# ZackAttack614/BlackBird

Hardware: AMD Instinct MI355X
Metric: selfplay_games_per_sec (higher is better)
Workload: dtype f32 (float32 operands split exactly into 3 bf16 values, 6 bf16 MFMA products each, f32 accumulate)

## Files before the change

### blackbird_amd/csrc/engine.hip

```cpp
#include "../../include/blackbird_hip.h"
#include "eval.hip.h"
#include "net.hip.h"
#include "net_x3.hip.h"
#include "gnet.hip.h"
#include "gnet_x3.hip.h"
#include "eval_probe.hip.h"
#include "tree.hip.h"
#include "tree_dc.hip.h"
#include "mega2.hip.h"
#include "mega_dc.hip.h"

#include <cmath>
#include <cstdarg>
#include <cstdio>
#include <cstdlib>
#include <cstring>
#include <string>
#include <type_traits>
#include <vector>

static thread_local std::string g_err;
static int fail(int code, const char *fmt, ...) {
    char buf[512];
    va_list ap;
// ... 154 lines not shown
    bb_game_info info;
    TreeDev dev;
    DCEdges edges;
    int32_t *d_child_action = nullptr;
    NetDev net;
    NetX3 x3 = {nullptr, nullptr, nullptr, nullptr, nullptr};
    size_t x3_bytes = 0;
    bool has_weights = false;
    int net_F = 0, net_C = 0;
    bool general_net = false;
    GNetDev gnet = {};
    GNetX3 gx3 = {nullptr, {nullptr, nullptr}};
    size_t gx3_bytes = 0;
    int gnet_C = 0;
    size_t net_sizes[4] = {0, 0, 0, 0};
    hipStream_t stream = nullptr;
    std::vector<void *> allocs;
    int n_games_target = 0;
    int sims_now = 0;
    size_t node_bytes = 0;
    double *d_u = nullptr;
    int32_t *d_actions = nullptr;
    int n_views = 1;
    TreeDev view[2];
    hipStream_t vstream[2] = {nullptr, nullptr};
    int vround[2] = {0, 0};
    struct {
        int launch_steps = 64, queue_limit_s = 30;
        bool level_budget_set = false;
    } tune;
    size_t eval_cache_bytes = 0;
    int *miss_count = nullptr;
    int *miss_slot = nullptr;
    int miss_next[2] = {0, 0};
    bool mega = false;
    bool async_selfplay = false;
    bool dc_fused = false;
    int round = 0;
    int time_every = 0;
    uint64_t eval_launches = 0;
    std::vector<hipEvent_t> ev_pool;
    size_t ev_used = 0;
};

static hipError_t sync_all(bb_engine *e) {
    if (e->vstream[1]) {
        hipError_t r = hipStreamSynchronize(e->vstream[1]);
        if (r != hipSuccess) return r;
    }
    return hipStreamSynchronize(e->stream);
}

template <class T>
static int dalloc(bb_engine *e, T *&p, size_t count, bool zero = true) {
    void *q = nullptr;
    size_t bytes = count * sizeof(T);
    hipError_t err = hipMalloc(&q, bytes ? bytes : 16);
    if (err != hipSuccess) return fail(BB_ERR_HIP, "hipMalloc(%zu) failed: %s", bytes, hipGetErrorString(err));
    e->allocs.push_back(q);
    if (zero && bytes) {
        err = hipMemsetAsync(q, 0, bytes, e->stream);
        if (err != hipSuccess) return fail(BB_ERR_HIP, "hipMemset failed: %s", hipGetErrorString(err));
    }
    p = (T *)q;
    return 0;
}
// ... 52 lines not shown
template <class G>
static void make_views(bb_engine *e) {
    const TreeDev &d = e->dev;
    int n = d.n_slots;
    for (int v = 0; v < e->n_views; v++) {
        TreeDev w = d;
        int off = v == 0 ? 0 : n / 2;
        int cnt = e->n_views == 1 ? n : (v == 0 ? n / 2 : n - n / 2);
        w.n_slots = cnt;
        w.slot_offset = off;
        w.root += off; w.root_N += off; w.n_nodes += off; w.ply += off; w.sims_left += off; w.pend_leaf += off;
        w.pend_expand += off; w.path_len += off; w.game_lid += off; w.sim_serial += off; w.root_W += off;
        w.root_pp += off; w.path += (size_t)off * G::MAXPATH;
        w.anc += (size_t)off * (d.max_plies + 2); w.anc_len += off; w.top_N += off;
        w.path_N += (size_t)off * G::MAXPATH; w.path_all += (size_t)off * G::MAXPATH; w.path_W += (size_t)off * G::MAXPATH; w.leaf_flags += off;
        w.leaf_state = (char *)d.leaf_state + (size_t)off * sizeof(typename G::State);
        w.leaf_game_id += off; w.leaf_serial += off; w.eval_value += off;
        w.eval_policy += (size_t)off * (G::GID == BB_GAME_DRAGONCHESS ? G::A : G::S);
        w.evals += off; w.ctr += (size_t)off * 8;
        w.nodes = (char *)d.nodes + (size_t)off * d.node_cap * e->node_bytes;
        w.resume_cur += off; w.resume_depth += off; w.post_slot += off; w.post_count += 4 * v;
        e->view[v] = w;
    }
}

static size_t eval_cache_entry_bytes(const bb_config *cfg) { return cfg->game == BB_GAME_DRAGONCHESS ? 128 : 64; }
static int eval_cache_log2_of(const bb_config *cfg) {
    const bool rounds_too = cfg->game == BB_GAME_CONNECT4;
    if ((cfg->game != BB_GAME_CONNECT4 && cfg->game != BB_GAME_DRAGONCHESS) || cfg->mcts_kind != BB_MCTS_DYNAMIC ||
        cfg->evaluator != BB_EVAL_NET || !(cfg->launch == BB_LAUNCH_AUTO || (rounds_too && cfg->launch == BB_LAUNCH_ROUNDS)))
        return 0;
    const char *on = getenv("BB_EVAL_CACHE"), *lg = getenv("BB_EVAL_CACHE_LOG2");
    if (on && atoi(on) == 0) return 0;
    const int k = lg ? atoi(lg) : cfg->game == BB_GAME_DRAGONCHESS ? 24 : 26;
    return k < 10 ? 10 : k > 32 ? 32 : k;
}

static long node_capacity_of(const bb_config *cfg) {
    long cap = cfg->node_capacity > 0 ? cfg->node_capacity : (long)cfg->sims_per_move * cfg->max_plies + 2;
    if (cfg->mcts_kind == BB_MCTS_FIXED && cfg->node_capacity <= 0) cap = cap * cfg->max_depth;
    return cap;
}

template <class G>
static void pool_bytes(const bb_config *cfg, size_t *per_slot, size_t *fixed) {
    constexpr bool DC = G::GID == BB_GAME_DRAGONCHESS;
    constexpr size_t NODE_BYTES = DC ? sizeof(DCNode) : sizeof(DenseNode<typename std::conditional<DC, Connect4, G>::type>);
    const size_t cap = (size_t)node_capacity_of(cfg);
    size_t ps = cap * NODE_BYTES;
    if (DC) ps += cap * 24 * sizeof(DCEdge) + (size_t)G::MAXPATH * 4;
    ps += (size_t)G::MAXPATH * 4 + (DC ? (size_t)G::A : (size_t)G::S) * 4 + (size_t)G::S * 16 + sizeof(typename G::State) + 256;
    bb_game_info gi;
    bb_game_info_get(cfg->game, &gi);
    const size_t ng = (size_t)(cfg->max_games > 0 ? cfg->max_games : cfg->n_slots);
    *per_slot = ps;
    *fixed = ng * ((size_t)(cfg->max_plies + 1) * (size_t)gi.example_bytes + 16) + (64u << 20);
    if (const int k = eval_cache_log2_of(cfg)) *fixed += eval_cache_entry_bytes(cfg) << k;
}

static int check_config(const bb_config *cfg) {
    if (!cfg) return fail(BB_ERR_ARG, "null argument");
    if (cfg->n_slots <= 0) return fail(BB_ERR_ARG, "n_slots must be positive");
    if (cfg->mcts_kind == BB_MCTS_FIXED && cfg->max_depth <= 0)
        return fail(BB_ERR_ARG, "MaxDepth for MCTS must be > 0.");
    if (cfg->sims_per_move < 0 || cfg->max_plies <= 0) return fail(BB_ERR_ARG, "bad sims_per_move/max_plies");
    int ndev = bb_device_count();
    if (ndev <= 0) return fail(BB_ERR_HIP, "no HIP device available (this library has no CPU fallback)");
// ... 71 lines not shown
    d.lid_stride = cfg->n_slots;
    auto env_int = [](const char *name, int dflt) {
        const char *v = getenv(name);
        return v ? atoi(v) : dflt;
    };
    if (int v = env_int("BB_LEVEL_BUDGET", 0); v >= 1) {
        d.level_budget = v;
        e->tune.level_budget_set = true;
    }
    e->tune.launch_steps = env_int("BB_LAUNCH_STEPS", 64);
    e->tune.queue_limit_s = env_int("BB_QUEUE_LIMIT_S", 30);
    if (cfg->launch < 0 || cfg->launch > BB_LAUNCH_ROUNDS || cfg->net_form < 0 || cfg->net_form > BB_NET_FORM_SPLIT) {
        delete e;
        return fail(BB_ERR_ARG, "bad bb_config.launch / net_form");
    }
    e->async_selfplay = cfg->game != BB_GAME_DRAGONCHESS && cfg->mcts_kind == BB_MCTS_DYNAMIC &&
                        cfg->evaluator != BB_EVAL_ROLLOUT && cfg->launch != BB_LAUNCH_LOCKSTEP;
    e->mega = e->async_selfplay && cfg->evaluator == BB_EVAL_NET && cfg->launch == BB_LAUNCH_AUTO;
    e->dc_fused = cfg->game == BB_GAME_DRAGONCHESS && cfg->mcts_kind == BB_MCTS_DYNAMIC && cfg->evaluator == BB_EVAL_NET &&
                  cfg->launch == BB_LAUNCH_AUTO;
    if (int v = env_int("BB_TREE_GPW", 0); v >= 1 && v <= 64 / e->info.S) d.gpw = v;
    d.temp = 1.0;
    GAME_SWITCH(cfg->game, rc = engine_alloc<G>(e); break);
    if (!rc) {
        if (const int k = eval_cache_log2_of(cfg)) {
            uint8_t *tab = nullptr;
            e->eval_cache_bytes = eval_cache_entry_bytes(cfg) << k;
            rc = dalloc(e, tab, e->eval_cache_bytes);
            d.eval_cache = tab;
            d.eval_cache_log2 = k;
        }
    }
    if (!rc) rc = dalloc(e, d.eval_cache_ctr, 2);
    if (!rc && d.eval_cache && e->async_selfplay) rc = dalloc(e, e->miss_count, 8) || dalloc(e, e->miss_slot, (size_t)cfg->n_slots);
    if (rc) {
        bb_destroy(e);
        return rc;
    }
    e->n_views = 1;
    if (e->async_selfplay && !e->mega && cfg->evaluator == BB_EVAL_NET && cfg->n_slots >= 512) e->n_views = 2;
    if (const char *env = getenv("BB_GROUPS")) e->n_views = (atoi(env) == 2 && e->async_selfplay && cfg->n_slots >= 2) ? 2 : 1;
    e->vstream[0] = e->stream;
    if (e->n_views == 2) HIPCHK(hipStreamCreateWithFlags(&e->vstream[1], hipStreamNonBlocking));
    GAME_SWITCH(cfg->game, make_views<G>(e); break);
    *out = e;
    return BB_OK;
}

extern "C" int bb_destroy(bb_engine *e) {
    if (!e) return BB_OK;
    (void)hipSetDevice(e->cfg.device);
    if (e->stream) (void)hipStreamSynchronize(e->stream);
    for (void *p : e->allocs) (void)hipFree(p);
    for (auto ev : e->ev_pool) (void)hipEventDestroy(ev);
    if (e->vstream[1]) {
        (void)hipStreamSynchronize(e->vstream[1]);
        (void)hipStreamDestroy(e->vstream[1]);
    }
    if (e->stream) (void)hipStreamDestroy(e->stream);
    delete e;
    return BB_OK;
}

extern "C" int bb_timing_enable(bb_engine *e, int every_n) {
    if (!e || every_n < 0) return fail(BB_ERR_ARG, "bad arguments");
    HIPCHK(hipSetDevice(e->cfg.device));
    HIPCHK(sync_all(e));
// ... 957 lines not shown
            if (e->x3.w0) {
                if constexpr (G::S <= 8) k_selfplay_queue<G, 8, true, 12><<<nb, 768, 0, e->stream>>>(dm, e->net, e->x3, e->cfg.noise_on, lim, own);
                else k_selfplay_queue<G, 4, true, 8><<<nb, 512, 0, e->stream>>>(dm, e->net, e->x3, e->cfg.noise_on, lim, own);
            } else {
                k_selfplay_queue<G, 8><<<nb, 768, 0, e->stream>>>(dm, e->net, e->x3, e->cfg.noise_on, lim, own);
            }
            HIPCHK(hipGetLastError());
            if (timed) {
                HIPCHK(hipEventRecord(e->ev_pool[e->ev_used + 1], e->stream));
                e->ev_used += 2;
            }
          }
            return BB_OK;
        }
        for (int r = 0; r < rounds; r++) {
            for (int v = 0; v < e->n_views; v++) {
                TreeDev &d = e->view[v];
                hipStream_t st = e->vstream[v];
                int tb = nblk((size_t)((d.n_slots + d.gpw - 1) / d.gpw) * 64);
                int nb = (d.n_slots + 4 * PWMAX - 1) / (4 * PWMAX);
                if (e->n_views == 2) nb = 256 > nb ? 256 : nb;
                int round = e->vround[v]++;
                k_tree_async<G><<<tb, 256, 0, st>>>(d, round);
                HIPCHK(hipGetLastError());
                const typename G::State *ls = (const typename G::State *)d.leaf_state;
                if (d.evaluator == BB_EVAL_NET) {
                    bool timed = v == 0 && e->time_every > 0 && (e->eval_launches++ % (uint64_t)e->time_every) == 0 &&
                                 e->ev_used + 2 <= e->ev_pool.size();
                    if (timed) HIPCHK(hipEventRecord(e->ev_pool[e->ev_used], st));
                    const int *n_ptr = d.post_count + (round & 3), *slot_list = d.post_slot;
                    EvalCache store = {nullptr, 0};
                    if constexpr (G::CACHE_KEY) {
                        if (d.eval_cache && e->miss_count && e->general_net) {
                            store = {(u32x4 *)d.eval_cache, d.eval_cache_log2};
                            int *mc = e->miss_count + 4 * v, *ms = e->miss_slot + d.slot_offset;
                            if (e->miss_next[v] != round)
                                HIPCHK(hipMemsetAsync(mc, 0, 4 * sizeof(int), st));
                            e->miss_next[v] = round + 1;
                            k_eval_cache_probe<G><<<(d.n_slots + 3) / 4, 256, 0, st>>>(e->net, store, n_ptr, slot_list, mc, round, ms, ls,
                                                                                       d.leaf_game_id, d.leaf_serial, e->cfg.noise_on,
                                                                                       d.eval_value, d.eval_policy, G::S, d.evals,
                                                                                       d.eval_cache_ctr);
                            n_ptr = mc + (round & 3);
                            slot_list = ms;
                        }
                    }
                    if (e->general_net) {
                        int rc = launch_gnet<G>(e, d.n_slots, n_ptr, slot_list, ls, nullptr, d.leaf_game_id,
                                                d.leaf_serial, e->cfg.noise_on, d.eval_value, nullptr, d.eval_policy, G::S, st,
                                                d.slot_offset, store);
                        if (rc) return rc;
                    } else if (e->x3.w0) {
                        if constexpr (G::C <= 4)
                            k_net_x3<G><<<(d.n_slots + 3) / 4, 256, 0, st>>>(e->net, e->x3, 0, n_ptr, slot_list, ls,
                                                                              nullptr, d.leaf_game_id, d.leaf_serial, e->cfg.noise_on,
                                                                              d.eval_value, nullptr, d.eval_policy, G::S, store);
                    } else
                    k_net_compact<G, PWMAX><<<nb, 256, 0, st>>>(e->net, n_ptr, slot_list, ls,
                                                                 d.leaf_game_id, d.leaf_serial, e->cfg.noise_on, d.eval_value,
                                                                 d.eval_policy, G::S, store);
                    HIPCHK(hipGetLastError());
                    if (timed) {
                        HIPCHK(hipEventRecord(e->ev_pool[e->ev_used + 1], st));
                        e->ev_used += 2;
                    }
                } else {
                    k_hash_eval<G><<<nblk(d.n_slots), 256, 0, st>>>(d.n_slots, ls, d.leaf_game_id, d.salt, d.salt_per_game,
                                                                    d.first_game_id, d.eval_value, d.eval_policy, G::S);
                    HIPCHK(hipGetLastError());
                }
            }
        }
// ... 260 lines not shown
```

### blackbird_amd/csrc/eval_probe.hip.h

```cpp
#pragma once
#include "net.hip.h"

template <class G>
__global__ void __launch_bounds__(256)
k_eval_cache_probe(NetDev nd, EvalCache cache, const int *n_ptr, const int *slot_list, int *miss_count, int round, int *miss_slot,
                   const typename G::State *states, const uint32_t *game_id, const int32_t *serial, int noise, float *value_out,
                   float *policy_out, int pstride, uint64_t *evals, unsigned long long *ctr) {
    static_assert(G::CACHE_KEY, "a game whose positions have a one-word key (Connect4)");
    __shared__ int s_slot[4], s_probe[4], s_base;
    const int wave = __builtin_amdgcn_readfirstlane(threadIdx.x >> 6), lane = threadIdx.x & 63;
    const int n = *n_ptr, pos = blockIdx.x * 4 + wave;
    const bool live = pos < n;
    const int slot = slot_list[live ? pos : 0];
    const typename G::State st = states[slot];
    const uint64_t key = live ? G::cache_key(st) : 0;
    u32x4 *const entry = eval_cache_entry(cache, key);
    const u32x4 chunk = eval_cache_load(entry, lane);
    if (blockIdx.x == 0 && threadIdx.x == 0) miss_count[(round + 2) & 3] = 0;
    float cv = 0.f, cpr = 0.f;
    const bool hit = eval_cache_hit<G::A>(chunk, key, lane, cv, cpr) && key != 0;
    if (hit) {
        if (lane == 0) {
            value_out[slot] = cv;
            evals[slot] -= 1;
        }
        dense_prior_tail<G>(nd, cpr, slot, true, game_id, serial, noise, policy_out, pstride, lane);
    }
    if (lane == 0) {
        s_slot[wave] = live && !hit ? slot : -1;
        s_probe[wave] = key ? 1 + (int)hit : 0;
    }
    __syncthreads();
    if (threadIdx.x == 0) {
        int n_miss = 0, n_probe = 0, n_hit = 0;
        for (int w = 0; w < 4; w++) {
            n_miss += s_slot[w] >= 0;
            n_probe += s_probe[w] > 0;
            n_hit += s_probe[w] > 1;
        }
        s_base = n_miss ? atomicAdd(&miss_count[round & 3], n_miss) : 0;
        if (n_probe && ctr) {
            if (n_hit) atomicAdd(&ctr[0], (unsigned long long)n_hit);
            atomicAdd(&ctr[1], (unsigned long long)n_probe);
        }
    }
    __syncthreads();
    if (lane == 0 && s_slot[wave] >= 0) {
        int rank = 0;
        for (int w = 0; w < wave; w++) rank += s_slot[w] >= 0;
        miss_slot[s_base + rank] = slot;
    }
}
```

### blackbird_amd/csrc/games.hip.h

```cpp
#pragma once
#include <hip/hip_runtime.h>
#include <stdint.h>

template <class T>
__device__ __forceinline__ T *as_lds(T *p) {
#if __HIP_DEVICE_COMPILE__
    __builtin_assume(__builtin_amdgcn_is_shared((const void *)p));
#endif
    return p;
}
template <class T>
__device__ __forceinline__ T *as_global(T *p) {
#if __HIP_DEVICE_COMPILE__
    __builtin_assume(!__builtin_amdgcn_is_shared((const void *)p) && !__builtin_amdgcn_is_private((const void *)p));
#endif
    return p;
}

struct GridState {
    uint64_t p1, p2;
};
static_assert(sizeof(GridState) == 16, "packed grid state is 16 bytes");

#define BB_HD __host__ __device__ __forceinline__
// ... 115 lines not shown
                for (int r = 0; r < H; r++) col |= 1ull << (r * STR);
                uint64_t cb = (occ >> prev) & col;
                int top = cb ? (63 - bb_clz64(cb)) / STR : 0;
                cell = top * STR + prev;
            } else {
                cell = (prev / W) * STR + (prev % W);
            }
            uint64_t bit = 1ull << cell;
            int p = (b1 & bit) ? 1 : (b2 & bit) ? 2 : 0;
            uint64_t own = p == 1 ? b1 : p == 2 ? b2 : (~occ & board_mask());
            if (win_cells(own) & bit) return p;
        } else {
            uint64_t w1 = win_cells(b1), w2 = win_cells(b2), any = w1 | w2;
            if (any) return (w1 >> bb_ctz64(any)) & 1 ? 1 : 2;
        }
        if (is_over(occ)) return 0;
        return -1;
    }

    BB_HD static void encode_cell(const State &s, int r, int c, int8_t out[3]) {
        int bit = r * STR + c;
        out[0] = (int8_t)((s.p1 >> bit) & 1);
        out[1] = (int8_t)((s.p2 >> bit) & 1);
        out[2] = gs_player(s) == 1 ? 1 : -1;
    }

    static constexpr bool CACHE_KEY = DROP;
    BB_HD static uint64_t cache_key(const State &s) {
        const uint64_t b1 = gs_cells(s.p1), b2 = gs_cells(s.p2), occ = b1 | b2, floor = (1ull << W) - 1;
        const uint64_t above = (occ << STR) | floor;
        if (!DROP || (b1 & b2) || (occ & ~board_mask()) || (occ & ~above)) return 0;
        return b1 | (above & ~occ) | ((uint64_t)(gs_player(s) == 1) << 63);
    }
};

BB_HD uint64_t bb_mix64(uint64_t z) {
    z ^= z >> 33;
    z *= 0xff51afd7ed558ccdull;
    z ^= z >> 33;
    z *= 0xc4ceb9fe1a85ec53ull;
    z ^= z >> 33;
    return z;
}

using Connect4 = GridGame<6, 7, 4, 8, 7, 8, 0>;
using TicTacToe = GridGame<3, 3, 3, 4, 9, 16, 1>;

struct alignas(16) DCState {
    int8_t b[64];
    int8_t player, prev;
    int8_t castle[4];
    int8_t pad[10];
};
static_assert(sizeof(DCState) == 80, "packed DragonChess state is 80 bytes");

struct DCKey {
    uint64_t w[5];
    BB_HD bool none() const { return (w[0] | w[1] | w[2] | w[3] | w[4]) == 0; }
    BB_HD bool operator==(const DCKey &o) const {
        return w[0] == o.w[0] && w[1] == o.w[1] && w[2] == o.w[2] && w[3] == o.w[3] && w[4] == o.w[4];
    }
    BB_HD uint64_t tag() const {
        uint64_t t = bb_mix64(w[0]);
        for (int i = 1; i < 5; i++) t = bb_mix64(t ^ w[i]);
        return t;
    }
};

struct DragonChess {
    static constexpr int H = 8, W = 8, C = 17, A = 4032, S = 144, GID = 2;
    static constexpr int MAXPATH = 128;
    static constexpr bool CELL_BF16 = true;
    static constexpr bool CACHE_KEY = false;
    using State = DCState;

    BB_HD static State initial() {
        State s;
        for (int i = 0; i < 64; i++) s.b[i] = 0;
        const int8_t back[8] = {-5, -3, -4, -6, -1, -4, -3, -5};
// ... 268 lines not shown
```

### blackbird_amd/csrc/net.hip.h

```cpp
#pragma once
#include <type_traits>
#include "games.hip.h"
#include "rng.hip.h"

typedef float f32x4 __attribute__((ext_vector_type(4)));

__device__ __forceinline__ void wave_lds_handover() { __builtin_amdgcn_fence(__ATOMIC_ACQ_REL, "wavefront"); }

struct NetDev {
    int R, D, A;
    const float *w0;
    const f32x4 *wt;
    const float *epi;
    const float *head;
    int head_floats;
    int off_vk, off_v3, off_d1k, off_d1b, off_d2k, off_d2b, off_pk, off_p6, off_pdk, off_pdb;
    uint64_t seed;
    float alpha, eps;
    float inv_alpha, inv_beta;
    int dbg;
};
#ifdef BB_DIAG
#define ND_DBG(bit) (nd.dbg & (bit))
#else
// ... 88 lines not shown
    float sv[NPL];
    float m = -INFINITY;
#pragma unroll
    for (int k0 = 0; k0 < NPL; k0 += UB) {
        float w0[UB], w1[UB], wb[UB];
#pragma unroll
        for (int u = 0; u < UB; u++) {
            const int a = lane + 64 * (k0 + u);
            w0[u] = pdk[a];
            w1[u] = pdk[A + a];
            wb[u] = pdb[a];
        }
#pragma unroll
        for (int u = 0; u < UB; u++) {
            sv[k0 + u] = wide_logit<HW>(h.R0, h.R1, w0[u], w1[u], wb[u]);
            m = fmaxf(m, sv[k0 + u]);
        }
    }
    m = wave_max_f32(m);
    float tot = 0.f;
#pragma unroll
    for (int k = 0; k < NPL; k++) tot += wide_expterm(sv[k], m);
    tot = wave_sum_f32(tot);
    h.m = m;
    h.inv = 1.0f / tot;
}

__device__ __forceinline__ float pooled_sum(float v) { return wave_sum_f32(v); }

typedef unsigned int u32x4 __attribute__((ext_vector_type(4)));
struct EvalCache {
    u32x4 *tab;
    int log2;
};
__device__ __forceinline__ u32x4 *eval_cache_entry(const EvalCache &c, uint64_t key) {
    return c.tab + 4 * (size_t)(bb_mix64(key) >> (64 - c.log2));
}
template <int A>
__device__ __forceinline__ void eval_cache_put(u32x4 *entry, uint64_t key, float value, float pr, int lane) {
    static_assert(A == 7, "an entry holds the value and seven priors");
    const int c = lane < 4 ? lane : 0;
    const float lo = __shfl(pr, c > 0 ? 2 * c - 1 : 0, 64), hi = __shfl(pr, 2 * c, 64);
    if (lane < 4)
        *(__attribute__((address_space(1))) u32x4 *)(void *)(entry + lane) =
            u32x4{(uint32_t)key, (uint32_t)(key >> 32), __float_as_uint(c == 0 ? value : lo), __float_as_uint(hi)};
}
__device__ __forceinline__ u32x4 eval_cache_load(const u32x4 *entry, int lane) {
    u32x4 z = {0u, 0u, 0u, 0u};
    if (lane < 4) z = *(const __attribute__((address_space(1))) u32x4 *)(const void *)(entry + lane);
    return z;
}
template <int A>
__device__ __forceinline__ bool eval_cache_hit(u32x4 ch, uint64_t key, int lane, float &value, float &pr) {
    const bool ok = lane < 4 && ch[0] == (uint32_t)key && ch[1] == (uint32_t)(key >> 32);
    if ((__ballot(ok) & 0xFull) != 0xFull) return false;
    const float f0 = __uint_as_float(ch[2]), f1 = __uint_as_float(ch[3]);
    value = lane_f32(f0, 0);
    const int i = (lane < A ? lane : 0) + 1;
    const float lo = __shfl(f0, i >> 1, 64), hi = __shfl(f1, i >> 1, 64);
    pr = lane < A ? ((i & 1) ? hi : lo) : 0.f;
    return true;
}

__device__ __forceinline__ u32x4 *dc_eval_cache_entry(const EvalCache &c, uint64_t tag) {
    return c.tab + 8 * (size_t)(tag >> (64 - c.log2));
}
__device__ __forceinline__ u32x4 dc_eval_cache_load(const u32x4 *entry, int lane) {
    u32x4 z = {0u, 0u, 0u, 0u};
    if (lane < 8) z = *(const __attribute__((address_space(1))) u32x4 *)(const void *)(entry + lane);
    return z;
}
__device__ __forceinline__ uint64_t dc_key_word(DCKey k, int lane) {
    return lane == 0 ? k.w[0] : lane == 1 ? k.w[1] : lane == 2 ? k.w[2] : lane == 3 ? k.w[3] : k.w[4];
}
__device__ __forceinline__ bool dc_eval_cache_hit(u32x4 ch, DCKey key, uint64_t tag, int lane, WideHead &h) {
    const uint64_t pay = (uint64_t)ch[2] | ((uint64_t)ch[3] << 32);
    const bool ok = lane < 8 && ch[0] == (uint32_t)tag && ch[1] == (uint32_t)(tag >> 32) && (lane >= 5 || pay == dc_key_word(key, lane));
    if ((__ballot(ok) & 0xFFull) != 0xFFull) return false;
    const float f0 = __uint_as_float(ch[2]), f1 = __uint_as_float(ch[3]);
    h.value = lane_f32(f0, 5);
    h.R0 = lane_f32(f1, 5);
    h.R1 = lane_f32(f0, 6);
    h.m = lane_f32(f1, 6);
    h.inv = lane_f32(f0, 7);
    return true;
}
__device__ __forceinline__ void dc_eval_cache_put(u32x4 *entry, DCKey key, uint64_t tag, WideHead h, int lane) {
    const uint64_t kw = dc_key_word(key, lane);
    const uint32_t lo = lane < 5 ? (uint32_t)kw : __float_as_uint(lane == 5 ? h.value : lane == 6 ? h.R1 : h.inv);
    const uint32_t hi = lane < 5 ? (uint32_t)(kw >> 32) : lane == 5 ? __float_as_uint(h.R0) : lane == 6 ? __float_as_uint(h.m) : 0u;
    if (lane < 8)
        *(__attribute__((address_space(1))) u32x4 *)(void *)(entry + lane) = u32x4{(uint32_t)tag, (uint32_t)(tag >> 32), lo, hi};
// ... 92 lines not shown
                    if (lane + 64 * k < A) {
                        sv[k] = (1.0f - nd.eps) * (sv[k] * inv) + nd.eps * bb_beta_noise(nd.seed, gid, ser, (uint32_t)(lane + 64 * k), nd.alpha);
                        t2 += sv[k];
                    }
                t2 = wave_sum_f32(t2);
                inv = 1.0f / t2;
            }
#pragma unroll
            for (int k = 0; k < NPL; k++)
                if (lane + 64 * k < A) outp[lane + 64 * k] = sv[k] * inv;
        }
    } else {
        static_assert(A > 64 || 2 * A <= 64, "the prior-noise draws use two lanes per action");
        const bool act = lane < A;
        const float l = act ? wide_logit<HW>(R0, R1, pdk[act ? lane : 0], pdk[A + (act ? lane : 0)], pdb[act ? lane : 0]) : -INFINITY;
        constexpr bool ROW0 = A <= 16;
        const float m = ROW0 ? row0_max_f32(l) : wave_max_f32(l);
        float pr = act ? wide_expterm(l, m) : 0.f;
        const float tot = ROW0 ? row0_sum_f32(pr) : wave_sum_f32(pr);
        pr = pr * __builtin_amdgcn_rcpf(tot);
        if constexpr (A == 7)
            if (cache_entry) eval_cache_put<A>(cache_entry, cache_key, value, pr, lane);
        if (live && act && logits_out) logits_out[(size_t)pos * A + lane] = l;
        dense_prior_tail<G>(nd, pr, pos, live, game_id, serial, noise, policy_out, pstride, lane);
    }
}

template <class G>
__device__ __forceinline__ u32x4 *eval_cache_store_entry(const EvalCache &store, const typename G::State *states, int pos, bool live,
                                                         uint64_t &key) {
    key = 0;
    if constexpr (G::CACHE_KEY) {
        if (store.tab && states && live) key = G::cache_key(states[pos]);
        if (key) return eval_cache_entry(store, key);
    }
    return nullptr;
}

template <class G, int PW>
__device__ __forceinline__ void net_head_tail(const NetDev &nd, int n, int pos0, const int *slot_list, const float *rv,
                                              const float *rp, const uint32_t *game_id, const int32_t *serial, int noise,
                                              float *value_out, float *logits_out, float *policy_out, int pstride,
                                              WideHead *compact = nullptr, EvalCache store = {nullptr, 0},
                                              const typename G::State *states = nullptr) {
    constexpr int HW = G::H * G::W;
    static_assert(HW <= 64, "one lane per pixel of a position");
    const int lane = threadIdx.x & 63;
    for (int pp = 0; pp < PW; pp++) {
        const bool live = pos0 + pp < n;
        if (!live && !compact) break;
        const int pos = live ? (slot_list ? slot_list[pos0 + pp] : pos0 + pp) : 0;
        const float x = lane < HW ? rv[pp * HW + lane] : 0.f;
        const float x0 = lane < HW ? rp[2 * (pp * HW + lane)] : 0.f, x1 = lane < HW ? rp[2 * (pp * HW + lane) + 1] : 0.f;
        uint64_t ckey;
        u32x4 *centry = eval_cache_store_entry<G>(store, states, pos, live, ckey);
        head_one<G>(nd, pooled_sum(x), pooled_sum(x0), pooled_sum(x1), pos, live, game_id, serial, noise, value_out, logits_out,
                    policy_out, pstride, compact ? compact + pp : nullptr, centry, ckey);
    }
}

template <class G, int PW, int WMODE = 0>
__device__ __forceinline__ void net_body(const NetDev &nd, int n, int pos0, const int *slot_list, float *wlds,
                                         const typename G::State *states, const int8_t *planes,
                                         const uint32_t *game_id, const int32_t *serial, int noise, float *value_out,
                                         float *logits_out, float *policy_out, int pstride, bool zero_lds = true,
                                         WideHead *compact = nullptr, EvalCache store = {nullptr, 0}) {
    using NG = NetGeom<G, PW>;
// ... 356 lines not shown
```

### blackbird_amd/csrc/net_x3.hip.h

```cpp
#pragma once
#include "net.hip.h"

typedef __bf16 bf16x8 __attribute__((ext_vector_type(8)));
typedef short s16x4 __attribute__((ext_vector_type(4)));
typedef unsigned int u32x2 __attribute__((ext_vector_type(2)));
typedef unsigned int u32x4 __attribute__((ext_vector_type(4)));

template <class G>
struct X3Geom {
    static constexpr int H = G::H, W = G::W, CIN = G::C, A = G::A, HW = H * W;
    static_assert(CIN <= 32, "the first conv packs at most 32 input planes per tap");
    static_assert(HW <= 64, "one lane per pixel in the heads");
    static constexpr bool WIDE_IN = CIN > 4;
    static constexpr int RS = W + 1;
    static constexpr int S0 = RS + 1;
    static constexpr bool CONTIG = (16 % RS) == 0;
    static_assert(CONTIG || (W == 8 && H % 2 == 0), "tile shapes exist for 4-, 8- and 9-slot rows");
    static constexpr int NT = CONTIG ? (H * RS + 15) / 16 : H / 2;
    static constexpr bool SWZ = RS == 8;
    static constexpr int SLOT_B = 96;
    static constexpr int SLOTS_BOARD = (H + 2) * RS + 2;
    static constexpr int SLOTS_TILES = CONTIG ? S0 + 16 * NT + RS + 2 : 0;
    static constexpr int SLOTS = SLOTS_BOARD > SLOTS_TILES ? SLOTS_BOARD : SLOTS_TILES;
    static constexpr int X_B = SLOTS * SLOT_B;
// ... 79 lines not shown
__device__ __forceinline__ void net_body_x3(const NetDev &nd, const NetX3 &x3, int n, int pos0, const int *slot_list,
                                            unsigned char *wl, const typename G::State *states, const int8_t *planes,
                                            const uint32_t *game_id, const int32_t *serial, int noise, float *value_out,
                                            float *logits_out, float *policy_out, int pstride, bool zero_lds,
                                            WideHead *compact = nullptr, EvalCache cache = {nullptr, 0}, int *probe_out = nullptr) {
    using XG = X3Geom<G>;
    constexpr int W = XG::W, CIN = XG::CIN, HW = XG::HW, NT = XG::NT, SB = XG::SLOT_B, RS = XG::RS;
    constexpr bool WIDE_IN = XG::WIDE_IN;
    int lane_ = threadIdx.x & 63;
    asm volatile("" : "+v"(lane_));
    const int lane = lane_;
    const int g = lane >> 4, nn = lane & 15, gh = g >> 1, gl = g & 1;
    static_assert(!PP || !WLDS, "the two-buffer form keeps its weights in registers, a layer ahead");
    unsigned char *X = wl;
    unsigned char *X2 = wl + XG::X_B;
    typename G::State *sst = (typename G::State *)(wl + (PP ? 2 : 1) * XG::X_B);
    auto OI = [&](int pos) { return slot_list ? slot_list[pos] : pos; };
    const bool live = pos0 < n;
#ifdef BB_STAMPS_NET
    long long _ns = clock64();
#endif

    const typename G::State *sst_in = sst;
    typename G::State my_state;
    if constexpr (PP) sst_in = as_lds(&states[OI(live ? pos0 : 0)]);
    else my_state = planes ? G::initial() : states[OI(live ? pos0 : 0)];
    static_assert(!CACHE || (G::CACHE_KEY && !PP), "the evaluation cache: Connect4, value and priors formed here");
    uint64_t ckey = 0;
    u32x4 *centry = nullptr;
    u32x4 cchunk = {0u, 0u, 0u, 0u};
    if constexpr (CACHE) {
        if (cache.tab && live && !planes) ckey = G::cache_key(my_state);
        if (ckey) {
            centry = eval_cache_entry(cache, ckey);
            cchunk = eval_cache_load(centry, lane);
        }
        if (probe_out) *probe_out = ckey ? 0 : -1;
    }
    const unsigned char *w0p = x3.w0;
    bf16x8 w0a[WIDE_IN ? 27 : 3];
    bf16x8 w0b;
    if constexpr (WIDE_IN) {
#pragma unroll
        for (int i = 0; i < 27; i++) w0a[i] = WLDS ? *(const bf16x8 *)(w0p + (i * 64 + lane) * 16) : x3_ldg(w0p + (i * 64 + lane) * 16);
    } else {
#pragma unroll
        for (int q = 0; q < 3; q++) w0a[q] = *(const bf16x8 *)(w0p + (q * 64 + lane) * 16);
        w0b = *(const bf16x8 *)(w0p + (3 * 64 + lane) * 16);
    }
    const float *epi = PP ? as_lds(nd.epi) : nd.epi;
    const f32x4 bias0 = *(const f32x4 *)(epi + 4 * g), scale0 = *(const f32x4 *)(epi + 16 + 4 * g),
                shift0 = *(const f32x4 *)(epi + 32 + 4 * g);
    NSUB(5);
    if (zero_lds) {
        u32x4 z = {0u, 0u, 0u, 0u};
        if constexpr (PP) {
            constexpr int NHALO = RS + XG::H + (XG::SLOTS - (XG::H + 1) * RS), CH = SB / 16;
            constexpr int NCH = 2 * NHALO * CH;
#pragma unroll
            for (int k = 0; k < (NCH + 63) / 64; k++) {
                const int i = lane + 64 * k;
                const int buf = i >= NHALO * CH, j = i - buf * NHALO * CH, hs = j / CH, c = j - hs * CH;
                const int slot = hs < RS ? hs : hs < RS + XG::H ? (hs - RS + 1) * RS : (XG::H + 1) * RS + (hs - RS - XG::H);
                if (64 * k + 63 < NCH || i < NCH) *(u32x4 *)(wl + buf * XG::X_B + slot * SB + c * 16) = z;
            }
        } else {
            for (int i = lane; i < XG::WAVE_BYTES / 16; i += 64) ((u32x4 *)wl)[i] = z;
// ... 28 lines not shown
                unsigned b[32];
#pragma unroll
                for (int c = 0; c < 32; c++) b[c] = c < CIN ? __float_as_uint((float)v[c]) >> 16 : 0u;
#pragma unroll
                for (int k = 0; k < 16; k++) pk[k] = b[2 * k] | (b[2 * k + 1] << 16);
            }
            unsigned char *dst = X + ((y + 1) * RS + (x + 1)) * SB;
#pragma unroll
            for (int k = 0; k < 4; k++) *(u32x4 *)(dst + 16 * k) = u32x4{pk[4 * k], pk[4 * k + 1], pk[4 * k + 2], pk[4 * k + 3]};
        }
    } else
    if (lane < HW && live) {
        const int y = lane / W, x = lane % W;
        int8_t v[4] = {0, 0, 0, 0};
        if (planes) {
            const int8_t *src = planes + ((size_t)pos0 * HW + lane) * CIN;
#pragma unroll
            for (int c = 0; c < CIN; c++) v[c] = src[c];
        } else {
            int8_t e[CIN];
            if constexpr (PP) G::encode_cell(*sst_in, y, x, e);
            else G::encode_cell(my_state, y, x, e);
#pragma unroll
            for (int c = 0; c < CIN; c++) v[c] = e[c];
        }
        unsigned b[4];
#pragma unroll
        for (int c = 0; c < 4; c++) b[c] = __float_as_uint((float)v[c]) >> 16;
        *(u32x2 *)(X + ((y + 1) * RS + (x + 1)) * SB) = u32x2{b[0] | (b[1] << 16), b[2] | (b[3] << 16)};
    }
    NSUB(7);
    if constexpr (CACHE) {
        float cv, cpr;
        if (centry && eval_cache_hit<G::A>(cchunk, ckey, lane, cv, cpr)) {
            if (probe_out) *probe_out = 1;
            if (lane == 0 && value_out) value_out[OI(pos0)] = cv;
            dense_prior_tail<G>(nd, cpr, OI(pos0), true, game_id, serial, noise, policy_out, pstride, lane);
            return;
        }
    }
    constexpr int TS = (XG::CONTIG ? 16 : 2 * RS) * SB;
    static_assert(XG::tile_slot(NT - 1, 5) * SB == XG::tile_slot(0, 5) * SB + (NT - 1) * TS && (!XG::SWZ || XG::swz(XG::tile_slot(1, 9)) == XG::swz(XG::tile_slot(0, 9))), "tile stride");
    auto tapoff = [](int tap) { return (tap / 3) * RS + (tap % 3); };
    const int t0off = tapoff(2 * g) * SB, t1off = tapoff(2 * g + 1) * SB;
    const int s0 = XG::tile_slot(0, nn);
    const int aA0 = (s0 - RS - 1 + gh) * SB + ((gl ^ XG::swz(s0 - 1 + gh)) << 4);
    const int aB0 = (s0 + (gh - 1) * RS + 1) * SB + ((gl ^ XG::swz(s0 + 1)) << 4);
    const int aC0 = (s0 + RS + 1) * SB + ((gl ^ XG::swz(s0 + 1)) << 4);
    const int aC1 = aC0 + gh * 32, aC3 = aC0 + (1 - gh) * 64;
    const int aO0 = s0 * SB + ((g ^ (XG::swz(s0) << 1)) << 3);
    const int aH0 = s0 * SB + ((gl ^ XG::swz(s0)) << 4);
    const int aH1 = aH0 + gh * 32, aH3 = aH0 + (1 - gh) * 64;
    const int iA0 = (s0 - RS - 1) * SB;
    bool wv[NT];
#pragma unroll
    for (int t = 0; t < NT; t++) wv[t] = XG::tile_valid(t, nn);
#define aA(t) (aA0 + (t) * TS)
#define aB(t) (aB0 + (t) * TS)
#define aC1(t) (aC1 + (t) * TS)
#define aC3(t) (aC3 + (t) * TS)
#define aO(t) (aO0 + (t) * TS)
#define aH1(t) (aH1 + (t) * TS)
#define aH3(t) (aH3 + (t) * TS)
#define iA(t) (iA0 + (t) * TS)
    wave_lds_handover();
    NSTAMP(0);
    f32x4 acc[NT], sk[NT];
    {
#pragma unroll
        for (int t = 0; t < NT; t++) acc[t] = bias0;
        if constexpr (WIDE_IN) {
#pragma unroll
// ... 324 lines not shown
        const unsigned char *whp = x3.wh;
        const bf16x8 h1 = PP ? x3_ldg(whp + (0 * 64 + lane) * 16) : *(const bf16x8 *)(whp + (0 * 64 + lane) * 16),
                     h2 = PP ? x3_ldg(whp + (1 * 64 + lane) * 16) : *(const bf16x8 *)(whp + (1 * 64 + lane) * 16),
                     h3 = PP ? x3_ldg(whp + (2 * 64 + lane) * 16) : *(const bf16x8 *)(whp + (2 * 64 + lane) * 16);
        const f32x4 hb = {hbias, 0.f, 0.f, 0.f};
        bf16x8 y1[NT], y3[NT];
#pragma unroll
        for (int t = 0; t < NT; t++) {
            y1[t] = *(const bf16x8 *)(X + aH1(t));
            y3[t] = *(const bf16x8 *)(X + aH3(t));
        }
        float xs = 0.f;
#pragma unroll
        for (int t = 0; t < NT; t++) {
            f32x4 a = hb;
            a = __builtin_amdgcn_mfma_f32_16x16x32_bf16(h3, y3[t], a, 0, 0, 0);
            a = __builtin_amdgcn_mfma_f32_16x16x32_bf16(h2, y1[t], a, 0, 0, 0);
            a = __builtin_amdgcn_mfma_f32_16x16x32_bf16(h1, y1[t], a, 0, 0, 0);
            const float v = fmaxf(__builtin_fmaf(a[0], hscale, hshift), 0.f);
            xs += (g < 3 && wv[t]) ? v : 0.f;
        }
        xs += dpp_f32(xs, 0);
        xs += dpp_f32(xs, 1);
        xs += dpp_f32(xs, 2);
        xs += dpp_f32(xs, 3);
        R = lane_f32(xs, 0);
        R0 = lane_f32(xs, 16);
        R1 = lane_f32(xs, 32);
    }
    NSTAMP(3);
    if constexpr (CACHE) {
        if (centry) {
            ckey = G::cache_key(states[OI(pos0)]);
            centry = eval_cache_entry(cache, ckey);
        }
    } else if constexpr (!PP) {
        centry = eval_cache_store_entry<G>(cache, planes ? nullptr : states, live ? OI(pos0) : 0, live, ckey);
    }
    head_one<G>(nd, R, R0, R1, live ? OI(pos0) : 0, live, game_id, serial, noise, value_out,
                logits_out, policy_out, pstride, compact, centry, ckey);
    NSTAMP(4);
}

#undef aA
#undef aB
#undef aC1
#undef aC3
#undef aO
#undef aH1
#undef aH3
#undef iA
template <class G>
__global__ void __launch_bounds__(256) k_net_x3(NetDev nd, NetX3 x3, int n, const int *n_ptr, const int *slot_list, const typename G::State *states,
                                                const int8_t *planes, const uint32_t *game_id, const int32_t *serial, int noise,
                                                float *value_out, float *logits_out, float *policy_out, int pstride, EvalCache store) {
    using XG = X3Geom<G>;
    __shared__ __attribute__((aligned(16))) unsigned char lds[4 * XG::WAVE_BYTES];
    const int wave = threadIdx.x >> 6;
    const int pos0 = blockIdx.x * 4 + wave;
    if (n_ptr) n = *n_ptr;
    if (pos0 >= n) return;
    net_body_x3<G, false>(nd, x3, n, pos0, slot_list, lds + wave * XG::WAVE_BYTES, states, planes, game_id, serial, noise, value_out,
                          logits_out, policy_out, pstride, true, nullptr, store);
}
```

Measured before the change: 9139.

## Make eval cache two-way set associative with stone-count replacement and double its size

Turns the direct-mapped Connect4 evaluation cache into two-way buckets. Probes load both ways (8 lanes), and on a miss a victim way is chosen, preferring an empty way and otherwise the entry with more stones. The chosen way is carried to the store path through a per-slot byte array or LDS, and the default table size doubles. The aim is a higher hit rate so fewer positions need full network evaluations, at the cost of more probe bandwidth, extra ballots and more memory.

```diff
diff --git a/blackbird_amd/csrc/engine.hip b/blackbird_amd/csrc/engine.hip
--- a/blackbird_amd/csrc/engine.hip
+++ b/blackbird_amd/csrc/engine.hip
@@ -210,6 +210,7 @@
     size_t eval_cache_bytes = 0;
     int *miss_count = nullptr;
     int *miss_slot = nullptr;
+    unsigned char *miss_way = nullptr;
     int miss_next[2] = {0, 0};
     bool mega = false;
     bool async_selfplay = false;
@@ -328,7 +329,7 @@
         return 0;
     const char *on = getenv("BB_EVAL_CACHE"), *lg = getenv("BB_EVAL_CACHE_LOG2");
     if (on && atoi(on) == 0) return 0;
-    const int k = lg ? atoi(lg) : cfg->game == BB_GAME_DRAGONCHESS ? 24 : 26;
+    const int k = lg ? atoi(lg) : cfg->game == BB_GAME_DRAGONCHESS ? 24 : 27;
     return k < 10 ? 10 : k > 32 ? 32 : k;
 }
 
@@ -466,7 +467,8 @@
         }
     }
     if (!rc) rc = dalloc(e, d.eval_cache_ctr, 2);
-    if (!rc && d.eval_cache && e->async_selfplay) rc = dalloc(e, e->miss_count, 8) || dalloc(e, e->miss_slot, (size_t)cfg->n_slots);
+    if (!rc && d.eval_cache && e->async_selfplay)
+        rc = dalloc(e, e->miss_count, 8) || dalloc(e, e->miss_slot, (size_t)cfg->n_slots) || dalloc(e, e->miss_way, (size_t)cfg->n_slots);
     if (rc) {
         bb_destroy(e);
         return rc;
@@ -1490,12 +1492,13 @@
                     EvalCache store = {nullptr, 0};
                     if constexpr (G::CACHE_KEY) {
                         if (d.eval_cache && e->miss_count && e->general_net) {
-                            store = {(u32x4 *)d.eval_cache, d.eval_cache_log2};
+                            store = {(u32x4 *)d.eval_cache, d.eval_cache_log2, e->miss_way + d.slot_offset};
                             int *mc = e->miss_count + 4 * v, *ms = e->miss_slot + d.slot_offset;
                             if (e->miss_next[v] != round)
                                 HIPCHK(hipMemsetAsync(mc, 0, 4 * sizeof(int), st));
                             e->miss_next[v] = round + 1;
-                            k_eval_cache_probe<G><<<(d.n_slots + 3) / 4, 256, 0, st>>>(e->net, store, n_ptr, slot_list, mc, round, ms, ls,
+                            k_eval_cache_probe<G><<<(d.n_slots + 3) / 4, 256, 0, st>>>(e->net, store, n_ptr, slot_list, mc, round, ms,
+                                                                                       e->miss_way + d.slot_offset, ls,
                                                                                        d.leaf_game_id, d.leaf_serial, e->cfg.noise_on,
                                                                                        d.eval_value, d.eval_policy, G::S, d.evals,
                                                                                        d.eval_cache_ctr);
diff --git a/blackbird_amd/csrc/eval_probe.hip.h b/blackbird_amd/csrc/eval_probe.hip.h
--- a/blackbird_amd/csrc/eval_probe.hip.h
+++ b/blackbird_amd/csrc/eval_probe.hip.h
@@ -4,6 +4,7 @@
 template <class G>
 __global__ void __launch_bounds__(256)
 k_eval_cache_probe(NetDev nd, EvalCache cache, const int *n_ptr, const int *slot_list, int *miss_count, int round, int *miss_slot,
+                   unsigned char *miss_way,
                    const typename G::State *states, const uint32_t *game_id, const int32_t *serial, int noise, float *value_out,
                    float *policy_out, int pstride, uint64_t *evals, unsigned long long *ctr) {
     static_assert(G::CACHE_KEY, "a game whose positions have a one-word key (Connect4)");
@@ -14,11 +15,12 @@
     const int slot = slot_list[live ? pos : 0];
     const typename G::State st = states[slot];
     const uint64_t key = live ? G::cache_key(st) : 0;
-    u32x4 *const entry = eval_cache_entry(cache, key);
-    const u32x4 chunk = eval_cache_load(entry, lane);
+    u32x4 *const bucket = eval_cache_bucket(cache, key);
+    const u32x4 chunk = eval_cache_load(bucket, lane);
     if (blockIdx.x == 0 && threadIdx.x == 0) miss_count[(round + 2) & 3] = 0;
     float cv = 0.f, cpr = 0.f;
-    const bool hit = eval_cache_hit<G::A>(chunk, key, lane, cv, cpr) && key != 0;
+    int way = 0;
+    const bool hit = eval_cache_hit<G>(chunk, key, lane, cv, cpr, way) && key != 0;
     if (hit) {
         if (lane == 0) {
             value_out[slot] = cv;
@@ -28,6 +30,7 @@
     }
     if (lane == 0) {
         s_slot[wave] = live && !hit ? slot : -1;
+        if (live && !hit) miss_way[slot] = (unsigned char)way;
         s_probe[wave] = key ? 1 + (int)hit : 0;
     }
     __syncthreads();
diff --git a/blackbird_amd/csrc/games.hip.h b/blackbird_amd/csrc/games.hip.h
--- a/blackbird_amd/csrc/games.hip.h
+++ b/blackbird_amd/csrc/games.hip.h
@@ -171,6 +171,14 @@
         if (!DROP || (b1 & b2) || (occ & ~board_mask()) || (occ & ~above)) return 0;
         return b1 | (above & ~occ) | ((uint64_t)(gs_player(s) == 1) << 63);
     }
+    BB_HD static int key_stones(uint64_t key) {
+        static_assert(H + 1 <= 8 && (H + 1) * STR <= 63, "three doubling steps reach the floor; bit 63 is the player");
+        uint64_t f = key & ~(1ull << 63);
+        f |= f >> STR;
+        f |= f >> (2 * STR);
+        f |= f >> (4 * STR);
+        return bb_popc64(f) - W;
+    }
 };
 
 BB_HD uint64_t bb_mix64(uint64_t z) {
@@ -184,6 +192,19 @@
 
 using Connect4 = GridGame<6, 7, 4, 8, 7, 8, 0>;
 using TicTacToe = GridGame<3, 3, 3, 4, 9, 16, 1>;
+
+template <class G>
+BB_HD int eval_cache_pick_way(uint64_t key, bool whole0, uint64_t occ0, bool whole1) {
+    if (!whole0) return 0;
+    if (!whole1) return 1;
+    return G::key_stones(key) <= G::key_stones(occ0) ? 0 : 1;
+}
+template <class G>
+BB_HD int eval_cache_pick_way_of(uint64_t key, const uint64_t k[8]) {
+    const bool whole0 = k[0] != 0 && k[1] == k[0] && k[2] == k[0] && k[3] == k[0];
+    const bool whole1 = k[4] != 0 && k[5] == k[4] && k[6] == k[4] && k[7] == k[4];
+    return eval_cache_pick_way<G>(key, whole0, k[0], whole1);
+}
 
 struct alignas(16) DCState {
     int8_t b[64];
diff --git a/blackbird_amd/csrc/net.hip.h b/blackbird_amd/csrc/net.hip.h
--- a/blackbird_amd/csrc/net.hip.h
+++ b/blackbird_amd/csrc/net.hip.h
@@ -144,9 +144,10 @@
 struct EvalCache {
     u32x4 *tab;
     int log2;
+    const unsigned char *way = nullptr;
 };
-__device__ __forceinline__ u32x4 *eval_cache_entry(const EvalCache &c, uint64_t key) {
-    return c.tab + 4 * (size_t)(bb_mix64(key) >> (64 - c.log2));
+__device__ __forceinline__ u32x4 *eval_cache_bucket(const EvalCache &c, uint64_t key) {
+    return c.tab + 8 * (size_t)(bb_mix64(key) >> (65 - c.log2));
 }
 template <int A>
 __device__ __forceinline__ void eval_cache_put(u32x4 *entry, uint64_t key, float value, float pr, int lane) {
@@ -157,19 +158,30 @@
         *(__attribute__((address_space(1))) u32x4 *)(void *)(entry + lane) =
             u32x4{(uint32_t)key, (uint32_t)(key >> 32), __float_as_uint(c == 0 ? value : lo), __float_as_uint(hi)};
 }
-__device__ __forceinline__ u32x4 eval_cache_load(const u32x4 *entry, int lane) {
+__device__ __forceinline__ u32x4 eval_cache_load(const u32x4 *bucket, int lane) {
     u32x4 z = {0u, 0u, 0u, 0u};
-    if (lane < 4) z = *(const __attribute__((address_space(1))) u32x4 *)(const void *)(entry + lane);
+    if (lane < 8) z = *(const __attribute__((address_space(1))) u32x4 *)(const void *)(bucket + lane);
     return z;
 }
-template <int A>
-__device__ __forceinline__ bool eval_cache_hit(u32x4 ch, uint64_t key, int lane, float &value, float &pr) {
-    const bool ok = lane < 4 && ch[0] == (uint32_t)key && ch[1] == (uint32_t)(key >> 32);
-    if ((__ballot(ok) & 0xFull) != 0xFull) return false;
+template <class G>
+__device__ __forceinline__ bool eval_cache_hit(u32x4 ch, uint64_t key, int lane, float &value, float &pr, int &way) {
+    constexpr int A = G::A;
+    const bool ok = lane < 8 && ch[0] == (uint32_t)key && ch[1] == (uint32_t)(key >> 32);
+    const unsigned m = (unsigned)__ballot(ok) & 0xFFu;
+    if ((m & 0x0Fu) != 0x0Fu && (m & 0xF0u) != 0xF0u) {
+        const uint64_t mine = (uint64_t)ch[0] | ((uint64_t)ch[1] << 32);
+        const uint64_t k0 = ((uint64_t)__builtin_amdgcn_readlane(ch[1], 0) << 32) | (uint32_t)__builtin_amdgcn_readlane(ch[0], 0);
+        const uint64_t k1 = ((uint64_t)__builtin_amdgcn_readlane(ch[1], 4) << 32) | (uint32_t)__builtin_amdgcn_readlane(ch[0], 4);
+        const unsigned w = (unsigned)__ballot(lane < 8 && mine != 0 && mine == (lane < 4 ? k0 : k1)) & 0xFFu;
+        way = eval_cache_pick_way<G>(key, (w & 0x0Fu) == 0x0Fu, k0, (w & 0xF0u) == 0xF0u);
+        return false;
+    }
+    const int o = (m & 0x0Fu) == 0x0Fu ? 0 : 4;
+    way = o >> 2;
     const float f0 = __uint_as_float(ch[2]), f1 = __uint_as_float(ch[3]);
-    value = lane_f32(f0, 0);
+    value = lane_f32(f0, o);
     const int i = (lane < A ? lane : 0) + 1;
-    const float lo = __shfl(f0, i >> 1, 64), hi = __shfl(f1, i >> 1, 64);
+    const float lo = __shfl(f0, o + (i >> 1), 64), hi = __shfl(f1, o + (i >> 1), 64);
     pr = lane < A ? ((i & 1) ? hi : lo) : 0.f;
     return true;
 }
@@ -328,7 +340,7 @@
     key = 0;
     if constexpr (G::CACHE_KEY) {
         if (store.tab && states && live) key = G::cache_key(states[pos]);
-        if (key) return eval_cache_entry(store, key);
+        if (key) return eval_cache_bucket(store, key) + 4 * (store.way ? store.way[pos] & 1 : 0);
     }
     return nullptr;
 }
diff --git a/blackbird_amd/csrc/net_x3.hip.h b/blackbird_amd/csrc/net_x3.hip.h
--- a/blackbird_amd/csrc/net_x3.hip.h
+++ b/blackbird_amd/csrc/net_x3.hip.h
@@ -135,7 +135,7 @@
     if constexpr (CACHE) {
         if (cache.tab && live && !planes) ckey = G::cache_key(my_state);
         if (ckey) {
-            centry = eval_cache_entry(cache, ckey);
+            centry = eval_cache_bucket(cache, ckey);
             cchunk = eval_cache_load(centry, lane);
         }
         if (probe_out) *probe_out = ckey ? 0 : -1;
@@ -230,12 +230,15 @@
     NSUB(7);
     if constexpr (CACHE) {
         float cv, cpr;
-        if (centry && eval_cache_hit<G::A>(cchunk, ckey, lane, cv, cpr)) {
+        int cway = 0;
+        if (centry && eval_cache_hit<G>(cchunk, ckey, lane, cv, cpr, cway)) {
             if (probe_out) *probe_out = 1;
             if (lane == 0 && value_out) value_out[OI(pos0)] = cv;
             dense_prior_tail<G>(nd, cpr, OI(pos0), true, game_id, serial, noise, policy_out, pstride, lane);
             return;
         }
+        static_assert(!WIDE_IN && XG::STATE_B >= 4, "the state area is free");
+        if (lane == 0) *(int *)sst = cway;
     }
     constexpr int TS = (XG::CONTIG ? 16 : 2 * RS) * SB;
     static_assert(XG::tile_slot(NT - 1, 5) * SB == XG::tile_slot(0, 5) * SB + (NT - 1) * TS && (!XG::SWZ || XG::swz(XG::tile_slot(1, 9)) == XG::swz(XG::tile_slot(0, 9))), "tile stride");
@@ -626,7 +629,7 @@
     if constexpr (CACHE) {
         if (centry) {
             ckey = G::cache_key(states[OI(pos0)]);
-            centry = eval_cache_entry(cache, ckey);
+            centry = eval_cache_bucket(cache, ckey) + 4 * (*(const int *)sst & 1);
         }
     } else if constexpr (!PP) {
         centry = eval_cache_store_entry<G>(cache, planes ? nullptr : states, live ? OI(pos0) : 0, live, ckey);
```

New measurement: 9419 (median of 6 runs). 1.03x the previous value.
